# JiuTongBro/vqnerf_release

Hardware: AMD Instinct MI355X
Metric: rays/sec (render) 800x800, 64+64 samples/ray, NeuS SDF 8x256 + colour 4x256 (higher is better)
Workload: dtype f32; 1 GPU; BASELINE configs[1], nerf/hotdog-shaped NeuS render: one whole 800x800 pin-hole view per rank per step (camera at distance 4, fov 0.6911), n_samples=64, n_importance=64, up_sample_steps=4, sdf 8x256; parallelism=views x1 (no data-path collective)

## Files before the change

vqnerf_release_amd/csrc/neus_mlp.hip:

```cpp
#include "neus_launch.h"
#include <stdlib.h>

using namespace eng;

#ifdef VQN_STAMPS
__device__ unsigned long long g_stamps[8];
#define VQN_STAMP_DECL unsigned long long st_[6] = {0, 0, 0, 0, 0, 0}; unsigned long long st_prev = __builtin_amdgcn_s_memtime(); const unsigned long long st_begin = st_prev;
#define VQN_STAMP(i) { const unsigned long long st_now = __builtin_amdgcn_s_memtime(); st_[i] += st_now - st_prev; st_prev = st_now; }
#define VQN_STAMP_FLUSH if (threadIdx.x == 0) { st_[5] = __builtin_amdgcn_s_memtime() - st_begin; for (int i_ = 0; i_ < 6; ++i_) atomicAdd(&g_stamps[i_], st_[i_]); atomicAdd(&g_stamps[6], 1ull); }
extern "C" int vqn_debug_read_stamps(unsigned long long* out, int reset) {
  if (hipMemcpyFromSymbol(out, HIP_SYMBOL(g_stamps), sizeof(unsigned long long) * 8) != hipSuccess) return -3;
  if (reset) { unsigned long long z[8] = {0, 0, 0, 0, 0, 0, 0, 0}; if (hipMemcpyToSymbol(HIP_SYMBOL(g_stamps), z, sizeof(z)) != hipSuccess) return -3; }
  return 0;
}
#else
#define VQN_STAMP_DECL
#define VQN_STAMP(i)
#define VQN_STAMP_FLUSH
#endif

#ifdef VQN_STAMPS
__device__ unsigned long long g_stamps2[16];
#define FS_DECL unsigned long long fs_[16] = {0, 0, 0, 0, 0, 0, 0, 0, 0, 0, 0, 0, 0, 0, 0, 0}; unsigned long long fs_prev = __builtin_amdgcn_s_memtime(); const unsigned long long fs_begin = fs_prev;
#define FS(i) { const unsigned long long fs_now = __builtin_amdgcn_s_memtime(); fs_[i] += fs_now - fs_prev; fs_prev = fs_now; }
#define FS_FLUSH if (threadIdx.x == 0) { fs_[14] = __builtin_amdgcn_s_memtime() - fs_begin; for (int i_ = 0; i_ < 15; ++i_) atomicAdd(&g_stamps2[i_], fs_[i_]); atomicAdd(&g_stamps2[15], 1ull); }
extern "C" int vqn_debug_read_stamps2(unsigned long long* out, int reset) {
  if (hipMemcpyFromSymbol(out, HIP_SYMBOL(g_stamps2), sizeof(unsigned long long) * 16) != hipSuccess) return -3;
  if (reset) { unsigned long long z[16] = {0}; if (hipMemcpyToSymbol(HIP_SYMBOL(g_stamps2), z, sizeof(z)) != hipSuccess) return -3; }
  return 0;
}
#else
#define FS_DECL
#define FS(i)
#define FS_FLUSH
#endif

namespace {

constexpr int E0 = 0;
constexpr int E_ROWS = 8;

template <bool FINE>
__global__ __launch_bounds__(256, 2) void neus_points_kernel(
    const SdfDesc sd, const ColDesc cd, const f32x4* __restrict__ wsdf, const f32x4* __restrict__ wcol,
    const float* __restrict__ rays_o, const float* __restrict__ rays_d, const float* __restrict__ zv,
    const float* __restrict__ pts_direct, const float* __restrict__ dirs_direct, const long P, const int S,
    f32x4* __restrict__ scratch, float* __restrict__ out_sdf, float* __restrict__ out_grad,
    float* __restrict__ out_rgb) {
  extern __shared__ __attribute__((aligned(16))) f32x4 lds[];
  const int MT = sd.max_tiles;
  const int X0 = E_ROWS, Y0 = E_ROWS + 4 * MT;
  Smalls<1>* sm = reinterpret_cast<Smalls<1>*>(lds + (size_t)(E_ROWS + 8 * MT) * 64);
  const int tid = threadIdx.x, lane = tid & 63, h = lane >> 5, p = lane & 31;
  const int wave = __builtin_amdgcn_readfirstlane(tid >> 6);
  const int n_lin = sd.n_lin;
  const int emb_tiles = (sd.emb_feats + 31) >> 5;
  const long n_tiles = (P + 31) >> 5;
  f32x4* save = FINE ? scratch + (size_t)blockIdx.x * (size_t)(n_lin - 1) * 4 * MT * 64 : nullptr;
  const int feat_slot = (n_lin - 2) * 4 * MT;

  VQN_STAMP_DECL
  for (long tile = blockIdx.x; tile < n_tiles; tile += gridDim.x) {
    const long p0 = tile << 5;
    VQN_STAMP(4)
    if (tid < 32)
      load_point<FINE>(p0 + tid, P, S, rays_o, rays_d, zv, pts_direct, dirs_direct, sm->pts[0] + tid * 3, sm->dirs[0] + tid * 3);
    __syncthreads();
    const float xs = sm->pts[0][p * 3 + 0] * sd.scale, ys = sm->pts[0][p * 3 + 1] * sd.scale, zs = sm->pts[0][p * 3 + 2] * sd.scale;
    for (int r = wave; r < sd.emb_rows; r += 4) {
      f32x4 v;
#pragma unroll
      for (int j = 0; j < 4; ++j) v[j] = emb_feat(row_feat(r, h, j), sd.emb_feats, xs, ys, zs);
      lds[(E0 + r) * 64 + lane] = v;
    }
    __syncthreads();

    VQN_STAMP(0)
    int cur = X0, oth = Y0;
    f32x4 pre[4];
    {
      const f32x4* wp0 = wsdf + sd.layers[0].w_off + (size_t)wave * sd.emb_rows * 64 + lane;
#pragma unroll
      for (int i = 0; i < 4; ++i) pre[i] = wp0[i * 64];
    }
    for (int l = 0; l < n_lin - 1; ++l) {
      const LayerDesc L = sd.layers[l];
      const f32x4* next_wp = nullptr;
      if (l + 1 < n_lin - 1)
        next_wp = wsdf + sd.layers[l + 1].w_off + (size_t)wave * (4 * L.n_out_tiles + ((l + 1 == sd.skip) ? sd.emb_rows : 0)) * 64 + lane;
      const KSegs ks = (l == 0) ? KSegs{E0, sd.emb_rows, 0, 0}
                                : KSegs{cur, 4 * sd.layers[l - 1].n_out_tiles, E0, (l == sd.skip) ? sd.emb_rows : 0};
      const int dst = (l == 0) ? X0 : oth;
      const bool do_save = FINE && (l < n_lin - 2);
      const f32x4* bp = wsdf + L.b_off;
      f32x4* sv = save + (size_t)l * 4 * MT * 64;
      gemm_tiles_chain(lds, ks, wsdf + L.w_off, L.n_out_tiles, wave, lane, pre, next_wp,
                 [&](int ot, f32x16& acc) { VQN_STAMP(2) init_bias(bp, ot, lane, acc); },
                 [&](int ot, const f32x16& acc) {
                   VQN_STAMP(1)
#pragma unroll
                   for (int rq = 0; rq < 4; ++rq) {
                     f32x4 v = acc_quad(acc, rq);
#pragma unroll
                     for (int j = 0; j < 4; ++j) v[j] = act_fwd<ACT_SOFTPLUS100>(v[j]);
                     lds[(dst + ot * 4 + rq) * 64 + lane] = v;
                     if (do_save) st_stream(sv + (ot * 4 + rq) * 64 + lane, v);
                   }
                 });
      VQN_STAMP(2)
      __syncthreads();
      VQN_STAMP(3)
      if (l == 0) { cur = X0; oth = Y0; } else { const int t = cur; cur = oth; oth = t; }
    }
    const int hid_rows = 4 * sd.layers[n_lin - 2].n_out_tiles;

    rowdot<1>(lds, cur, hid_rows, wsdf + sd.last_w_off, sm->part[0], wave, lane);
    if (FINE && sd.layers[n_lin - 1].n_out_tiles > 0) {
      const LayerDesc L = sd.layers[n_lin - 1];
      const f32x4* bp = wsdf + L.b_off;
      f32x4* sv = save + (size_t)feat_slot * 64;
      gemm_tiles(lds, KSegs{cur, hid_rows, 0, 0}, wsdf + L.w_off, L.n_out_tiles, wave, lane,
                 [&](int ot, f32x16& acc) { init_bias(bp, ot, lane, acc); },
                 [&](int ot, const f32x16& acc) {
#pragma unroll
                   for (int rq = 0; rq < 4; ++rq) st_stream(sv + (ot * 4 + rq) * 64 + lane, acc_quad(acc, rq));
                 });
    }
    __syncthreads();
    if (tid < 32 && p0 + tid < P) out_sdf[p0 + tid] = sdf_raw(sm->part[0], tid, sd.last_b_off, sd.last_bias, wsdf) / sd.scale;
    if (!FINE) { __syncthreads(); continue; }

    for (int r0 = wave; r0 < hid_rows; r0 += 32) {
      f32x4 v[8], wv[8];
#pragma unroll
      for (int c = 0; c < 8; ++c) {
        const int r = min(r0 + 4 * c, hid_rows - 1);
        v[c] = lds[(cur + r) * 64 + lane];
        wv[c] = wsdf[sd.last_w_off + r * 2 + h];
      }
#pragma unroll
      for (int c = 0; c < 8; ++c)
        if (r0 + 4 * c < hid_rows) {
#pragma unroll
          for (int j = 0; j < 4; ++j) v[c][j] = wv[c][j] * act_bwd_from_out<ACT_SOFTPLUS100>(v[c][j]);
          lds[(cur + r0 + 4 * c) * 64 + lane] = v[c];
        }
    }
    __syncthreads();
    for (int l = n_lin - 2; l >= 1; --l) {
      const LayerDesc L = sd.layers[l];
      const KSegs ks{cur, 4 * L.n_out_tiles, 0, 0};
      const f32x4* sv = save + (size_t)(l - 1) * 4 * MT * 64;
      const int dst = oth;
      f32x4 hv[4];
      gemm_tiles(lds, ks, wsdf + L.wT_off, sd.layers[l - 1].n_out_tiles, wave, lane,
                 [&](int ot, f32x16& acc) {
#pragma unroll
                   for (int rq = 0; rq < 4; ++rq) hv[rq] = ld_stream(sv + (ot * 4 + rq) * 64 + lane);
                   init_zero(acc);
                 },
                 [&](int ot, const f32x16& acc) {
#pragma unroll
                   for (int rq = 0; rq < 4; ++rq) {
                     f32x4 v = acc_quad(acc, rq);
#pragma unroll
                     for (int j = 0; j < 4; ++j) v[j] *= act_bwd_from_out<ACT_SOFTPLUS100>(hv[rq][j]);
                     lds[(dst + ot * 4 + rq) * 64 + lane] = v;
                   }
                 });
      if (l == sd.skip)
        gemm_tiles(lds, ks, wsdf + L.wTE_off, emb_tiles, wave, lane,
                   [&](int, f32x16& acc) { init_zero(acc); },
                   [&](int ot, const f32x16& acc) {
#pragma unroll
                     for (int rq = 0; rq < 4; ++rq) lds[(E0 + ot * 4 + rq) * 64 + lane] = acc_quad(acc, rq);
                   });
      __syncthreads();
      const int t = cur; cur = oth; oth = t;
    }
    {
      const LayerDesc L = sd.layers[0];
      const bool accumulate = sd.skip >= 1;
      gemm_tiles(lds, KSegs{cur, 4 * L.n_out_tiles, 0, 0}, wsdf + L.wTE_off, emb_tiles, wave, lane,
                 [&](int ot, f32x16& acc) {
                   if (accumulate) init_rows(lds + (E0 + ot * 4) * 64, lane, acc); else init_zero(acc);
                 },
                 [&](int ot, const f32x16& acc) {
#pragma unroll
                   for (int rq = 0; rq < 4; ++rq) lds[(E0 + ot * 4 + rq) * 64 + lane] = acc_quad(acc, rq);
                 });
    }
    __syncthreads();
    if (tid < 96) {
      const int pp = tid & 31, c = tid >> 5;
      const float g = embed_chain([&](int f) { return lds_feat(lds, E0, f, pp); }, c, sd.multires, sm->pts[0] + pp * 3, sd.scale);
      sm->grad[0][pp * 3 + c] = g;
      if (p0 + pp < P) out_grad[(p0 + pp) * 3 + c] = g;
    }
    __syncthreads();
    if (cd.n_lin == 0) continue;

    {
      const float px = sm->pts[0][p * 3 + 0], py = sm->pts[0][p * 3 + 1], pz = sm->pts[0][p * 3 + 2];
      const float dx = sm->dirs[0][p * 3 + 0], dy = sm->dirs[0][p * 3 + 1], dz = sm->dirs[0][p * 3 + 2];
      for (int r = wave; r < cd.extra_rows; r += 4) {
        f32x4 v;
#pragma unroll
        for (int j = 0; j < 4; ++j) v[j] = col_extra_feat(row_feat(r, h, j), px, py, pz, dx, dy, dz, sm->grad[0] + p * 3, cd.n_view_feats, cd.extra_feats);
        lds[(E0 + r) * 64 + lane] = v;
      }
      const f32x4* sv = save + (size_t)feat_slot * 64;
      const int feat_rows = 4 * sd.layers[n_lin - 1].n_out_tiles;
      for (int r0 = wave; r0 < feat_rows; r0 += 32) {
        f32x4 v[8];
#pragma unroll
        for (int c = 0; c < 8; ++c) v[c] = ld_stream(sv + min(r0 + 4 * c, feat_rows - 1) * 64 + lane);
#pragma unroll
        for (int c = 0; c < 8; ++c)
          if (r0 + 4 * c < feat_rows) lds[(X0 + r0 + 4 * c) * 64 + lane] = v[c];
      }
      __syncthreads();
      cur = X0; oth = Y0;
      int in_rows = feat_rows;
      for (int l = 0; l < cd.n_lin - 1; ++l) {
        const LayerDesc L = cd.layers[l];
        const KSegs ks{cur, in_rows, E0, l == 0 ? cd.extra_rows : 0};
        const f32x4* bp = wcol + L.b_off;
        const int dst = oth;
        gemm_tiles(lds, ks, wcol + L.w_off, L.n_out_tiles, wave, lane,
                   [&](int ot, f32x16& acc) { init_bias(bp, ot, lane, acc); },
                   [&](int ot, const f32x16& acc) {
#pragma unroll
                     for (int rq = 0; rq < 4; ++rq) {
                       f32x4 v = acc_quad(acc, rq);
#pragma unroll
                       for (int j = 0; j < 4; ++j) v[j] = act_fwd<ACT_RELU>(v[j]);
                       lds[(dst + ot * 4 + rq) * 64 + lane] = v;
                     }
                   });
        __syncthreads();
        const int t = cur; cur = oth; oth = t;
        in_rows = 4 * L.n_out_tiles;
      }
      rowdot<3>(lds, cur, in_rows, wcol + cd.last_w_off, sm->part[0], wave, lane);
      __syncthreads();
      if (tid < 96) {
        const int pp = tid & 31, o = tid >> 5;
        const float v = rgb_out(sm->part[0], pp, o, cd.last_b_off, cd.last_bias[o], cd.squeeze_out, wcol);
        if (p0 + pp < P) out_rgb[(p0 + pp) * 3 + o] = v;
      }
    }
    __syncthreads();
  }
  VQN_STAMP(4)
  VQN_STAMP_FLUSH
}

__device__ __forceinline__ void wte_split_k(f32x4* __restrict__ lds, const int IS, const int k_row0, const int ng,
                                            const f32x4* __restrict__ w, const int emb_tiles, const int tmp_row0, const int tmp_rows,
                                            const int e_row0, const bool accumulate, const int wave, const int lane) {
  const int KS = min(8, tmp_rows >> 2) / emb_tiles, gk = (ng + KS - 1) / KS;
  const int t = wave % emb_tiles, kq = wave / emb_tiles;
  if (kq < KS) {
    f32x16 acc0, acc1;
    init_zero(acc0); init_zero(acc1);
    const int g0 = kq * gk, g1 = min(ng, g0 + gk);
    const f32x4* __restrict__ wp = w + (size_t)t * ng * 64 + lane;
    for (int g = g0; g < g1; g += 8) {
      f32x4 a[8], p[8], q[8];
#pragma unroll
      for (int i = 0; i < 8; ++i) {
        const int gg = min(g + i, ng - 1), r = (k_row0 + gg) * 64 + lane;
        a[i] = wp[gg * 64]; p[i] = lds[r]; q[i] = lds[r + IS];
      }
#pragma unroll
      for (int i = 0; i < 8; ++i)
        if (g + i < g1) {
#pragma unroll
          for (int j = 0; j < 4; ++j) {
            acc0 = __builtin_amdgcn_mfma_f32_32x32x2f32(a[i][j], p[i][j], acc0, 0, 0, 0);
            acc1 = __builtin_amdgcn_mfma_f32_32x32x2f32(a[i][j], q[i][j], acc1, 0, 0, 0);
          }
        }
    }
#pragma unroll
    for (int rq = 0; rq < 4; ++rq) {
      lds[(tmp_row0 + wave * 4 + rq) * 64 + lane] = acc_quad(acc0, rq);
      lds[IS + (tmp_row0 + wave * 4 + rq) * 64 + lane] = acc_quad(acc1, rq);
    }
  }
  __syncthreads();
  for (int r = wave; r < 8 * emb_tiles; r += 8) {
    const int im = r / (4 * emb_tiles), er = r - im * 4 * emb_tiles, tt = er >> 2, rq = er & 3;
    f32x4* li = lds + (size_t)im * IS;
    f32x4 sum = li[(tmp_row0 + tt * 4 + rq) * 64 + lane];
    for (int k = 1; k < KS; ++k) sum += li[(tmp_row0 + (k * emb_tiles + tt) * 4 + rq) * 64 + lane];
    if (accumulate) sum += li[(e_row0 + er) * 64 + lane];
    li[(e_row0 + er) * 64 + lane] = sum;
  }
  __syncthreads();
}

template <bool FINE, bool TRAIN = false, bool FOLD = false>
__global__ __launch_bounds__(512, 1) void neus_points2_kernel(
    const SdfDesc sd, const ColDesc cd, const f32x4* __restrict__ wsdf, const f32x4* __restrict__ wcol,
    const float* __restrict__ rays_o, const float* __restrict__ rays_d, const float* __restrict__ zv,
    const float* __restrict__ pts_direct, const float* __restrict__ dirs_direct, const long P, const int S,
    f32x4* __restrict__ scratch, float* __restrict__ out_sdf, float* __restrict__ out_grad,
    float* __restrict__ out_rgb, const TrainOut to) {
  extern __shared__ __attribute__((aligned(16))) f32x4 lds[];
  const int MT = sd.max_tiles;
  const int IMG = E_ROWS + 8 * MT, IS = IMG * 64;
  const int X0 = E_ROWS, Y0 = E_ROWS + 4 * MT;
  Smalls<2>* sm = reinterpret_cast<Smalls<2>*>(lds + (size_t)2 * IS);
  const int tid = threadIdx.x, lane = tid & 63, h = lane >> 5, p = lane & 31;
  const int wave = __builtin_amdgcn_readfirstlane(tid >> 6);
  const int img = wave >> 2, w4 = wave & 3;
  f32x4* ldsi = lds + (size_t)img * IS;
  const int n_lin = sd.n_lin;
  const int emb_tiles = (sd.emb_feats + 31) >> 5;
  const long n_tiles = (P + 31) >> 5, n_pairs = (n_tiles + 1) >> 1;
  const size_t per_img = (size_t)(n_lin - 1) * 4 * MT * 64;
#ifdef VQN_DIAG_STASH_ROT
  f32x4* save0 = nullptr;
#else
  f32x4* save0 = FINE ? scratch + (size_t)blockIdx.x * 2 * per_img : nullptr;
#endif
  const int feat_slot = (n_lin - 2) * 4 * MT;
  constexpr bool fold = FOLD;
  static_assert(!FOLD || (FINE && !TRAIN), "the fold is an inference path: the backward and the weight gradients read OUTF");
  f32x4 pre[4];
  f32x4 nopre[4];

  FS_DECL
  for (long pair = blockIdx.x; pair < n_pairs; pair += gridDim.x) {
#ifdef VQN_DIAG_STASH_ROT
    if (FINE) save0 = scratch + ((size_t)((pair / gridDim.x) % VQN_DIAG_STASH_ROT) * gridDim.x + blockIdx.x) * 2 * per_img;
#endif
    FS(12)
    if (tid < 64) {
      const int im = tid >> 5, t = tid & 31;
      load_point<FINE>(((2 * pair + im) << 5) + t, P, S, rays_o, rays_d, zv, pts_direct, dirs_direct, sm->pts[im] + t * 3, sm->dirs[im] + t * 3);
    }
    __syncthreads();
    const float xs = sm->pts[img][p * 3 + 0] * sd.scale, ys = sm->pts[img][p * 3 + 1] * sd.scale, zs = sm->pts[img][p * 3 + 2] * sd.scale;
    const long ptile_w = 2 * pair + img;
    for (int r = w4; r < (TRAIN ? 4 * to.e_tiles : sd.emb_rows); r += 4) {
      f32x4 v;
#pragma unroll
      for (int j = 0; j < 4; ++j) v[j] = r < sd.emb_rows ? emb_feat(row_feat(r, h, j), sd.emb_feats, xs, ys, zs) : 0.f;
      if (r < sd.emb_rows) ldsi[(E0 + r) * 64 + lane] = v;
      if (TRAIN && ptile_w < n_tiles) tfmt_store_quad(to.E, ptile_w, to.e_tiles, r >> 2, r & 3, lane, v);
    }
    __syncthreads();

    FS(0)
    int cur = X0, oth = Y0;
    if (wave < sd.layers[0].n_out_tiles) {
      const f32x4* wp0 = wsdf + sd.layers[0].w_off + (size_t)wave * sd.emb_rows * 64 + lane;
#pragma unroll
      for (int i = 0; i < 4; ++i) pre[i] = wp0[min(i, sd.emb_rows - 1) * 64];
    }
    for (int l = 0; l < n_lin - 1; ++l) {
      const LayerDesc L = sd.layers[l];
      const f32x4* next_wp = nullptr;
      if (l + 1 < n_lin - 1 && wave < sd.layers[l + 1].n_out_tiles)
        next_wp = wsdf + sd.layers[l + 1].w_off + (size_t)wave * (4 * L.n_out_tiles + ((l + 1 == sd.skip) ? sd.emb_rows : 0)) * 64 + lane;
      const KSegs ks = (l == 0) ? KSegs{E0, sd.emb_rows, 0, 0}
                                : KSegs{cur, 4 * sd.layers[l - 1].n_out_tiles, E0, (l == sd.skip) ? sd.emb_rows : 0};
      const int dst = (l == 0) ? X0 : oth;
      const bool do_save = FINE && (l < n_lin - 2);
      const f32x4* bp = wsdf + L.b_off;
      float* const t_u = TRAIN ? to.U[l + 1] : nullptr;
      auto bias_init = [&](int ot, int im, f32x16& acc) { if (im == 0) { FS(2) } init_bias(bp, ot, lane, acc); };
      auto epi_rq = [&](int ot, int im, int rq, const f32x16& acc) {
        if (im == 0 && rq == 0) { FS(1) }
        f32x4* li = lds + (size_t)im * IS;
        f32x4* sv = save0 + (size_t)im * per_img + (size_t)l * 4 * MT * 64;
        f32x4 v = {acc[4 * rq], acc[4 * rq + 1], acc[4 * rq + 2], acc[4 * rq + 3]};
#pragma unroll
        for (int j = 0; j < 4; ++j) v[j] = act_fwd<ACT_SOFTPLUS100>(v[j]);
        li[(dst + ot * 4 + rq) * 64 + lane] = v;
        if (do_save) st_stream(sv + (ot * 4 + rq) * 64 + lane, v);
        if (TRAIN && 2 * pair + im < n_tiles) tfmt_store_quad(t_u, 2 * pair + im, L.n_out_tiles, ot, rq, lane, v);
      };
      gemm_tiles2<8>(lds, IS, ks, wsdf + L.w_off, L.n_out_tiles, wave, lane, pre, true, next_wp, bias_init, epi_rq);
      FS(2)
      __syncthreads();
      FS(3)
      if (l == 0) { cur = X0; oth = Y0; } else { const int t = cur; cur = oth; oth = t; }
    }
    const int hid_rows = 4 * sd.layers[n_lin - 2].n_out_tiles;

    rowdot<1>(ldsi, cur, hid_rows, wsdf + sd.last_w_off, sm->part[img], w4, lane);
    if (FINE && sd.layers[n_lin - 1].n_out_tiles > 0) {
      const LayerDesc L = sd.layers[n_lin - 1];
      const f32x4* bp = fold ? wcol + cd.reserved2 : wsdf + L.b_off;
      gemm_tiles2<8>(lds, IS, KSegs{cur, hid_rows, 0, 0}, fold ? wcol + cd.reserved1 : wsdf + L.w_off,
                     fold ? cd.layers[0].n_out_tiles : L.n_out_tiles, wave, lane, nopre, false, nullptr,
                     [&](int ot, int, f32x16& acc) { init_bias(bp, ot, lane, acc); },
                     [&](int ot, int im, int rq, const f32x16& acc) {
                       f32x4* sv = save0 + (size_t)im * per_img + (size_t)feat_slot * 64;
                       const f32x4 v = {acc[4 * rq], acc[4 * rq + 1], acc[4 * rq + 2], acc[4 * rq + 3]};
                       st_stream(sv + (ot * 4 + rq) * 64 + lane, v);
                       if (TRAIN && 2 * pair + im < n_tiles) {
                         float* base = to.OUTF + (2 * pair + im) * (long)to.outf_tiles * 1024;
#pragma unroll
                         for (int j = 0; j < 4; ++j) {
                           const int f = 32 * ot + 2 * (4 * rq + j) + h + 1;
                           if (f < 32 * to.outf_tiles) __builtin_nontemporal_store(v[j], base + f * 32 + p);
                         }
                       }
                     });
    }
    __syncthreads();
    if (tid < 64) {
      const int im = tid >> 5, t = tid & 31;
      const long pt = ((2 * pair + im) << 5) + t;
      if (pt < P) out_sdf[pt] = sdf_raw(sm->part[im], t, sd.last_b_off, sd.last_bias, wsdf) / sd.scale;
      if (TRAIN && 2 * pair + im < n_tiles) {
        float* base = to.OUTF + (2 * pair + im) * (long)to.outf_tiles * 1024;
        base[t] = sdf_raw(sm->part[im], t, sd.last_b_off, sd.last_bias, wsdf);
        for (int f = 32 * sd.layers[n_lin - 1].n_out_tiles + 1; f < 32 * to.outf_tiles; ++f) base[f * 32 + t] = 0.f;
      }
    }
    if (!FINE) { __syncthreads(); FS(4) continue; }
    FS(4)

    float* const t_gh_top = TRAIN ? to.GH[n_lin - 2] : nullptr;
    for (int r0 = w4; r0 < hid_rows; r0 += 32) {
      f32x4 v[8], wv[8];
#pragma unroll
      for (int c = 0; c < 8; ++c) {
        const int r = min(r0 + 4 * c, hid_rows - 1);
        v[c] = ldsi[(cur + r) * 64 + lane];
        wv[c] = wsdf[sd.last_w_off + r * 2 + h];
      }
#pragma unroll
      for (int c = 0; c < 8; ++c)
        if (r0 + 4 * c < hid_rows) {
#pragma unroll
          for (int j = 0; j < 4; ++j) v[c][j] = wv[c][j] * act_bwd_from_out<ACT_SOFTPLUS100>(v[c][j]);
          ldsi[(cur + r0 + 4 * c) * 64 + lane] = v[c];
          if (TRAIN && ptile_w < n_tiles)
            tfmt_store_quad(t_gh_top, ptile_w, sd.layers[n_lin - 2].n_out_tiles, (r0 + 4 * c) >> 2, (r0 + 4 * c) & 3, lane, v[c]);
        }
    }
    __syncthreads();
    FS(5)
    for (int l = n_lin - 2; l >= 1; --l) {
      const LayerDesc L = sd.layers[l];
      const KSegs ks{cur, 4 * L.n_out_tiles, 0, 0};
      const int dst = oth;
      if (l == sd.skip)
        wte_split_k(lds, IS, cur, 4 * L.n_out_tiles, wsdf + L.wTE_off, emb_tiles, oth, 4 * MT, E0, false, wave, lane);
      f32x4 hv[2][4];
      float* const t_gh = TRAIN ? to.GH[l - 1] : nullptr;
      const int gh_tiles = sd.layers[l - 1].n_out_tiles;
      gemm_tiles2<8>(lds, IS, ks, wsdf + L.wT_off, sd.layers[l - 1].n_out_tiles, wave, lane, nopre, false, nullptr,
                     [&](int ot, int im, f32x16& acc) {
                       if (im == 0) { FS(7) }
                       const f32x4* sv = save0 + (size_t)im * per_img + (size_t)(l - 1) * 4 * MT * 64;
#pragma unroll
                       for (int rq = 0; rq < 4; ++rq) hv[im][rq] = ld_stream(sv + (ot * 4 + rq) * 64 + lane);
                       init_zero(acc);
                     },
                     [&](int ot, int im, int rq, const f32x16& acc) {
                       if (im == 0 && rq == 0) { FS(6) }
                       f32x4* li = lds + (size_t)im * IS;
                       f32x4 v = {acc[4 * rq], acc[4 * rq + 1], acc[4 * rq + 2], acc[4 * rq + 3]};
#pragma unroll
                       for (int j = 0; j < 4; ++j) v[j] *= act_bwd_from_out<ACT_SOFTPLUS100>(hv[im][rq][j]);
                       li[(dst + ot * 4 + rq) * 64 + lane] = v;
                       if (TRAIN && 2 * pair + im < n_tiles) tfmt_store_quad(t_gh, 2 * pair + im, gh_tiles, ot, rq, lane, v);
                     });
      FS(7)
      __syncthreads();
      FS(8)
      const int t = cur; cur = oth; oth = t;
    }
    wte_split_k(lds, IS, cur, 4 * sd.layers[0].n_out_tiles, wsdf + sd.layers[0].wTE_off, emb_tiles, oth, 4 * MT, E0, sd.skip >= 1, wave, lane);
    FS(6)
    if (tid < 192) {
      const int im = tid / 96, r = tid - 96 * im, pp = r & 31, c = r >> 5;
      const f32x4* li = lds + (size_t)im * IS;
      const float g = embed_chain([&](int f) { return lds_feat(li, E0, f, pp); }, c, sd.multires, sm->pts[im] + pp * 3, sd.scale);
      sm->grad[im][pp * 3 + c] = g;
      const long pt = ((2 * pair + im) << 5) + pp;
      if (pt < P) out_grad[pt * 3 + c] = g;
    }
    __syncthreads();
    FS(9)
    if (cd.n_lin == 0) continue;

    {
      const float px = sm->pts[img][p * 3 + 0], py = sm->pts[img][p * 3 + 1], pz = sm->pts[img][p * 3 + 2];
      const float dx = sm->dirs[img][p * 3 + 0], dy = sm->dirs[img][p * 3 + 1], dz = sm->dirs[img][p * 3 + 2];
      for (int r = w4; r < (TRAIN ? 4 * to.extr_tiles : cd.extra_rows); r += 4) {
        f32x4 v;
#pragma unroll
        for (int j = 0; j < 4; ++j)
          v[j] = r < cd.extra_rows ? col_extra_feat(row_feat(r, h, j), px, py, pz, dx, dy, dz, sm->grad[img] + p * 3, cd.n_view_feats, cd.extra_feats) : 0.f;
        if (r < cd.extra_rows) ldsi[(E0 + r) * 64 + lane] = v;
        if (TRAIN && ptile_w < n_tiles) tfmt_store_quad(to.EXTR, ptile_w, to.extr_tiles, r >> 2, r & 3, lane, v);
      }
      const f32x4* sv = save0 + (size_t)img * per_img + (size_t)feat_slot * 64;
      const int feat_rows = 4 * sd.layers[n_lin - 1].n_out_tiles;
      for (int r0 = w4; r0 < (fold ? 0 : feat_rows); r0 += 32) {
        f32x4 v[8];
#pragma unroll
        for (int c = 0; c < 8; ++c) v[c] = ld_stream(sv + min(r0 + 4 * c, feat_rows - 1) * 64 + lane);
#pragma unroll
        for (int c = 0; c < 8; ++c)
          if (r0 + 4 * c < feat_rows) ldsi[(X0 + r0 + 4 * c) * 64 + lane] = v[c];
      }
      __syncthreads();
      FS(10)
      cur = X0; oth = Y0;
      int in_rows = feat_rows;
      if (fold) {
        const LayerDesc L = cd.layers[0];
        const int dst = oth;
        gemm_tiles2<8>(lds, IS, KSegs{E0, cd.extra_rows, 0, 0}, wcol + cd.reserved3, L.n_out_tiles, wave, lane, nopre, false, nullptr,
                       [&](int ot, int im, f32x16& acc) {
                         const f32x4* pp = save0 + (size_t)im * per_img + (size_t)feat_slot * 64 + ot * 256 + lane;
#pragma unroll
                         for (int rq = 0; rq < 4; ++rq) {
                           const f32x4 v = ld_stream(pp + rq * 64);
                           acc[4 * rq + 0] = v[0]; acc[4 * rq + 1] = v[1]; acc[4 * rq + 2] = v[2]; acc[4 * rq + 3] = v[3];
                         }
                       },
                       [&](int ot, int im, int rq, const f32x16& acc) {
                         f32x4* li = lds + (size_t)im * IS;
                         f32x4 v = {acc[4 * rq], acc[4 * rq + 1], acc[4 * rq + 2], acc[4 * rq + 3]};
#pragma unroll
                         for (int j = 0; j < 4; ++j) v[j] = act_fwd<ACT_RELU>(v[j]);
                         li[(dst + ot * 4 + rq) * 64 + lane] = v;
                       });
        __syncthreads();
        const int t = cur; cur = oth; oth = t;
        in_rows = 4 * L.n_out_tiles;
      }
      for (int l = fold ? 1 : 0; l < cd.n_lin - 1; ++l) {
        const LayerDesc L = cd.layers[l];
        const KSegs ks{cur, in_rows, E0, l == 0 ? cd.extra_rows : 0};
        const f32x4* bp = wcol + L.b_off;
        const int dst = oth;
        float* const t_c = TRAIN ? to.C[l + 1] : nullptr;
        gemm_tiles2<8>(lds, IS, ks, wcol + L.w_off, L.n_out_tiles, wave, lane, nopre, false, nullptr,
                       [&](int ot, int, f32x16& acc) { init_bias(bp, ot, lane, acc); },
                       [&](int ot, int im, int rq, const f32x16& acc) {
                         f32x4* li = lds + (size_t)im * IS;
                         f32x4 v = {acc[4 * rq], acc[4 * rq + 1], acc[4 * rq + 2], acc[4 * rq + 3]};
#pragma unroll
                         for (int j = 0; j < 4; ++j) v[j] = act_fwd<ACT_RELU>(v[j]);
                         li[(dst + ot * 4 + rq) * 64 + lane] = v;
                         if (TRAIN && 2 * pair + im < n_tiles) tfmt_store_quad(t_c, 2 * pair + im, L.n_out_tiles, ot, rq, lane, v);
                       });
        __syncthreads();
        const int t = cur; cur = oth; oth = t;
        in_rows = 4 * L.n_out_tiles;
      }
      FS(11)
      rowdot<3>(ldsi, cur, in_rows, wcol + cd.last_w_off, sm->part[img], w4, lane);
      __syncthreads();
      if (tid < 192) {
        const int im = tid / 96, r = tid - 96 * im, pp = r & 31, o = r >> 5;
        const float v = rgb_out(sm->part[im], pp, o, cd.last_b_off, cd.last_bias[o], cd.squeeze_out, wcol);
        const long pt = ((2 * pair + im) << 5) + pp;
        if (pt < P) out_rgb[pt * 3 + o] = v;
      }
    }
    __syncthreads();
  }
  FS(12)
  FS_FLUSH
}

template <int NIMG>
struct SmallsSdf {
  float pts[NIMG][96], dirs[NIMG][96], part[NIMG][128];
};

template <int NIMG>
__global__ __launch_bounds__(512, 1) void neus_pointsN_kernel(
    const SdfDesc sd, const f32x4* __restrict__ wsdf, const float* __restrict__ rays_o, const float* __restrict__ rays_d,
    const float* __restrict__ zv, const float* __restrict__ pts_direct, const long P, const int S, float* __restrict__ out_sdf) {
  extern __shared__ __attribute__((aligned(16))) f32x4 lds[];
  const int MT = sd.max_tiles;
  const int X0 = sd.emb_rows, IS = (sd.emb_rows + 4 * MT) * 64;
  SmallsSdf<NIMG>* sm = reinterpret_cast<SmallsSdf<NIMG>*>(lds + (size_t)NIMG * IS);
  const int tid = threadIdx.x, lane = tid & 63, h = lane >> 5, p = lane & 31;
  const int wave = __builtin_amdgcn_readfirstlane(tid >> 6);
  const int n_lin = sd.n_lin;
  const long n_tiles = (P + 31) >> 5, n_groups = (n_tiles + NIMG - 1) / NIMG;
  f32x4 pre[4];
  f32x16 acc[NIMG];

  for (long grp = blockIdx.x; grp < n_groups; grp += gridDim.x) {
    if (tid < 32 * NIMG) {
      const int im = tid >> 5, t = tid & 31;
      load_point<false>(((NIMG * grp + im) << 5) + t, P, S, rays_o, rays_d, zv, pts_direct, nullptr, sm->pts[im] + t * 3, sm->dirs[im] + t * 3);
    }
    __syncthreads();
    for (int u = wave; u < NIMG * sd.emb_rows; u += 8) {
      const int im = u / sd.emb_rows, r = u - im * sd.emb_rows;
      const float xs = sm->pts[im][p * 3 + 0] * sd.scale, ys = sm->pts[im][p * 3 + 1] * sd.scale, zs = sm->pts[im][p * 3 + 2] * sd.scale;
      f32x4 v;
#pragma unroll
      for (int j = 0; j < 4; ++j) v[j] = emb_feat(row_feat(r, h, j), sd.emb_feats, xs, ys, zs);
      lds[(size_t)im * IS + (E0 + r) * 64 + lane] = v;
    }
    __syncthreads();

    if (wave < sd.layers[0].n_out_tiles) {
      const f32x4* wp0 = wsdf + sd.layers[0].w_off + (size_t)wave * sd.emb_rows * 64 + lane;
#pragma unroll
      for (int i = 0; i < 4; ++i) pre[i] = wp0[min(i, sd.emb_rows - 1) * 64];
    }
    for (int l = 0; l < n_lin - 1; ++l) {
      const LayerDesc L = sd.layers[l];
      const f32x4* next_wp = nullptr;
      if (l + 1 < n_lin - 1 && wave < sd.layers[l + 1].n_out_tiles)
        next_wp = wsdf + sd.layers[l + 1].w_off + (size_t)wave * (4 * L.n_out_tiles + ((l + 1 == sd.skip) ? sd.emb_rows : 0)) * 64 + lane;
      const KSegs ks = (l == 0) ? KSegs{E0, sd.emb_rows, 0, 0}
                                : KSegs{X0, 4 * sd.layers[l - 1].n_out_tiles, E0, (l == sd.skip) ? sd.emb_rows : 0};
      const f32x4* bp = wsdf + L.b_off;
      gemm_tilesN<NIMG, 8>(lds, IS, ks, wsdf + L.w_off, L.n_out_tiles, wave, lane, pre, next_wp, acc,
                           [&](int ot, int, f32x16& a) { init_bias(bp, ot, lane, a); },
                           [&](int, int, int rq, f32x16& a) {
#pragma unroll
                             for (int j = 0; j < 4; ++j) a[4 * rq + j] = act_fwd<ACT_SOFTPLUS100>(a[4 * rq + j]);
                           });
      if (l > 0) __syncthreads();
      if (wave < L.n_out_tiles) {
#pragma unroll
        for (int im = 0; im < NIMG; ++im) {
#pragma unroll
          for (int rq = 0; rq < 4; ++rq) lds[(size_t)im * IS + (X0 + wave * 4 + rq) * 64 + lane] = acc_quad(acc[im], rq);
        }
      }
      __syncthreads();
    }
    const int hid_rows = 4 * sd.layers[n_lin - 2].n_out_tiles;

    for (int u = wave; u < 4 * NIMG; u += 8)
      rowdot<1>(lds + (size_t)(u >> 2) * IS, X0, hid_rows, wsdf + sd.last_w_off, sm->part[u >> 2], u & 3, lane);
    __syncthreads();
    if (tid < 32 * NIMG) {
      const int im = tid >> 5, t = tid & 31;
      const long pt = ((NIMG * grp + im) << 5) + t;
      if (pt < P) out_sdf[pt] = sdf_raw(sm->part[im], t, sd.last_b_off, sd.last_bias, wsdf) / sd.scale;
    }
    __syncthreads();
  }
}

int check_sdf_desc(const SdfDesc& d) {
  if (d.n_lin < 2 || d.n_lin > VQN_MAX_SDF_LAYERS) return 1;
  if (d.max_tiles < 1 || d.max_tiles > 16) return 2;
  if (d.emb_feats < 3 || d.emb_feats > 64 || d.emb_rows < 1 || d.emb_rows > 8) return 3;
  if (d.skip >= d.n_lin - 1 || d.skip == 0) return 4;
  for (int l = 0; l < d.n_lin; ++l)
    if (d.layers[l].n_out_tiles < 0 || d.layers[l].n_out_tiles > d.max_tiles) return 5;
  if (!(d.scale > 0.f)) return 6;
  return 0;
}

template <int NIMG>
size_t lds_bytes(int MT) { return (size_t)NIMG * (E_ROWS + 8 * MT) * 1024 + sizeof(Smalls<NIMG>); }

bool use_two_images(int MT) {
  static const bool forced32 = getenv("VQN_NEUS_TILE32") != nullptr;
  return !forced32 && MT >= 5 && lds_bytes<2>(MT) <= 160 * 1024;
}

template <int NIMG>
size_t lds_bytes_sdf(const SdfDesc& sd) { return (size_t)NIMG * (sd.emb_rows + 4 * sd.max_tiles) * 1024 + sizeof(SmallsSdf<NIMG>); }

constexpr int SDF_IMAGES_DEFAULT = 4;
int sdf_images(const SdfDesc& sd) {
  static const int cap = [] {
    const char* e = getenv("VQN_NEUS_SDF_IMAGES");
    const int v = e != nullptr ? atoi(e) : SDF_IMAGES_DEFAULT;
    return v >= 2 && v <= 4 ? v : SDF_IMAGES_DEFAULT;
  }();
  if (!use_two_images(sd.max_tiles)) return 1;
  if (sd.max_tiles <= 8) {
    if (cap >= 4 && lds_bytes_sdf<4>(sd) <= 160 * 1024) return 4;
    if (cap >= 3 && lds_bytes_sdf<3>(sd) <= 160 * 1024) return 3;
  }
  return 2;
}

template <int NIMG>
int launch_sdf_images(const char* fn, const SdfDesc& sd, const f32x4* ws, const float* rays_o, const float* rays_d, const float* z,
                      const float* pts, const int64_t P, const int S, float* out_sdf, void* stream) {
  return vqn_launch(fn, neus_pointsN_kernel<NIMG>, pair_grid((P + 31) / 32, NIMG, 0, 0), 512, lds_bytes_sdf<NIMG>(sd), stream, sd, ws,
                    rays_o, rays_d, z, pts, (long)P, S, out_sdf);
}

bool extras_rows_ok(const ColDesc& cd) { return cd.extra_rows >= 1 && cd.extra_rows <= 8; }

}

extern "C" int vqn_neus_sdf_points(const int32_t* sdf_desc, const float* wbuf_sdf, const float* rays_o,
                                   const float* rays_d, const float* z, const float* pts, int64_t P, int S,
                                   float* out_sdf, void* stream) {
  SdfDesc sd;
  const int rc = neus_sdf_args(__func__, sdf_desc, wbuf_sdf, rays_o, rays_d, z, pts, P, S, out_sdf, check_sdf_desc,
                               "invalid SDF network descriptor", &sd);
  if (rc != VQN_OK || P == 0) return rc;
  ColDesc cd;
  memset(&cd, 0, sizeof(cd));
  const long n_tiles = (P + 31) / 32;
  const f32x4* ws = reinterpret_cast<const f32x4*>(wbuf_sdf);
  const int images = sdf_images(sd);
  if (images == 4) return launch_sdf_images<4>(__func__, sd, ws, rays_o, rays_d, z, pts, P, S, out_sdf, stream);
  if (images == 3) return launch_sdf_images<3>(__func__, sd, ws, rays_o, rays_d, z, pts, P, S, out_sdf, stream);
  if (images == 2)
    return vqn_launch(__func__, neus_points2_kernel<false>, pair_grid(n_tiles, 2, 0, 0), 512, lds_bytes<2>(sd.max_tiles), stream, sd, cd, ws,
                      nullptr, rays_o, rays_d, z, pts, nullptr, (long)P, S, nullptr, out_sdf, nullptr, nullptr, TrainOut{});
  const size_t lds = lds_bytes<1>(sd.max_tiles);
  VQN_CHECK_SHAPE(lds <= 160 * 1024, "network too wide for LDS");
  return vqn_launch(__func__, neus_points_kernel<false>, pair_grid(n_tiles, 1, 0, 0), 256, lds, stream, sd, cd, ws, nullptr, rays_o, rays_d,
                    z, pts, nullptr, (long)P, S, nullptr, out_sdf, nullptr, nullptr);
}

extern "C" int vqn_neus_train_fwd(const int32_t* sdf_desc, const float* wbuf_sdf, const int32_t* col_desc, const float* wbuf_col,
                                  const float* pts, const float* dirs, int64_t P, void* scratch, int64_t scratch_bytes,
                                  float* const* tensors, int n_tensors, int e_tiles, int outf_tiles, int extr_tiles, float* out_sdf,
                                  float* out_n, float* out_rgb, void* stream) {
  VQN_CHECK_ARG(sdf_desc && wbuf_sdf && col_desc && wbuf_col && pts && dirs && scratch && tensors && out_sdf && out_n && out_rgb, "null pointer");
  VQN_CHECK_ARG(P >= 1, "P >= 1");
  SdfDesc sd;
  ColDesc cd;
  memcpy(&sd, sdf_desc, sizeof(SdfDesc));
  memcpy(&cd, col_desc, sizeof(ColDesc));
  VQN_CHECK_SHAPE(check_sdf_desc(sd) == 0, "invalid SDF network descriptor");
  VQN_CHECK_SHAPE(cd.n_lin >= 2 && cd.n_lin <= VQN_MAX_COL_LAYERS && cd.d_out == 3 && sd.layers[sd.n_lin - 1].n_out_tiles >= 1, "colour net");
  VQN_CHECK_SHAPE(use_two_images(sd.max_tiles), "the training forward kernel is the two-image form only");
  const int nL = sd.n_lin - 1, nC = cd.n_lin - 1;
  VQN_CHECK_ARG(n_tensors == 3 + 2 * nL + nC, "tensors: [E, OUTF, EXTR, U_1..U_nL, GH_0..GH_{nL-1}, C_1..C_nC]");
  VQN_CHECK_SHAPE(e_tiles * 4 >= sd.emb_rows && e_tiles <= 2 && extr_tiles * 4 >= cd.extra_rows && extr_tiles <= 2 &&
                  outf_tiles >= sd.layers[sd.n_lin - 1].n_out_tiles, "tile counts");
  for (int i = 0; i < n_tensors; ++i) VQN_CHECK_ARG(tensors[i] != nullptr, "null tensor pointer");
  const long grid = pair_grid((P + 31) / 32, 2, neus_stash_bytes(sd), scratch_bytes);
  VQN_CHECK_ARG(grid >= 1, "scratch too small (see vqn_neus_fine_scratch_bytes)");
  return vqn_launch(__func__, neus_points2_kernel<true, true>, grid, 512, lds_bytes<2>(sd.max_tiles), stream, sd, cd,
                    reinterpret_cast<const f32x4*>(wbuf_sdf), reinterpret_cast<const f32x4*>(wbuf_col), nullptr, nullptr, nullptr, pts, dirs,
                    (long)P, 1, reinterpret_cast<f32x4*>(scratch), out_sdf, out_n, out_rgb,
                    neus_train_out(tensors, nL, nC, e_tiles, outf_tiles, extr_tiles));
}

extern "C" int64_t vqn_neus_fine_scratch_bytes(const int32_t* sdf_desc) {
  if (!sdf_desc) return -1;
  SdfDesc sd;
  memcpy(&sd, sdf_desc, sizeof(SdfDesc));
  const int emb_rows = sd.emb_rows;
  if (emb_rows >= 1 && emb_rows <= 12) sd.emb_rows = 1;
  if (check_sdf_desc(sd) != 0) return -2;
#ifdef VQN_DIAG_STASH_ROT
  return (int64_t)VQN_DIAG_STASH_ROT * vqn_num_cus() * 2 * neus_stash_bytes(sd);
#else
  return (int64_t)vqn_num_cus() * 2 * neus_stash_bytes(sd);
#endif
}

extern "C" int vqn_neus_fine_points(const int32_t* sdf_desc, const float* wbuf_sdf, const int32_t* col_desc,
                                    const float* wbuf_col, const float* rays_o, const float* rays_d, const float* z,
                                    const float* pts, const float* dirs, int64_t P, int S, void* scratch,
                                    int64_t scratch_bytes, float* out_sdf, float* out_grad, float* out_rgb,
                                    void* stream) {
  SdfDesc sd;
  ColDesc cd;
  const int rc = neus_fine_args(__func__, sdf_desc, wbuf_sdf, col_desc, wbuf_col, rays_o, rays_d, z, pts, dirs, P, S, scratch, out_sdf,
                                out_grad, out_rgb, check_sdf_desc, "invalid SDF network descriptor", extras_rows_ok, &sd, &cd);
  if (rc != VQN_OK || P == 0) return rc;
  if (cd.n_lin != 0)
    VQN_CHECK_ARG((cd.reserved1 > 0 && cd.reserved2 > cd.reserved1 && cd.reserved3 > cd.reserved2) ||
                  (cd.reserved1 == 0 && cd.reserved2 == 0 && cd.reserved3 == 0), "col_desc: fold offsets (reserved1..3) inconsistent");
  const long n_tiles = (P + 31) / 32;
  const int64_t per_img = neus_stash_bytes(sd);
  const f32x4* ws = reinterpret_cast<const f32x4*>(wbuf_sdf);
  const f32x4* wc = reinterpret_cast<const f32x4*>(wbuf_col);
  if (use_two_images(sd.max_tiles)) {
    const bool fold = cd.n_lin != 0 && cd.reserved1 > 0;
#ifdef VQN_DIAG_STASH_ROT
    const long grid = pair_grid(n_tiles, 2, 0, 0);
    VQN_CHECK_ARG((int64_t)VQN_DIAG_STASH_ROT * grid * 2 * per_img <= scratch_bytes, "diag build: scratch must hold ROT regions per workgroup");
#else
    const long grid = pair_grid(n_tiles, 2, per_img, scratch_bytes);
#endif
    VQN_CHECK_ARG(grid >= 1, "scratch too small (see vqn_neus_fine_scratch_bytes)");
    return vqn_launch(__func__, fold ? neus_points2_kernel<true, false, true> : neus_points2_kernel<true>, grid, 512, lds_bytes<2>(sd.max_tiles),
                      stream, sd, cd, ws, wc, rays_o, rays_d, z, pts, dirs, (long)P, S, reinterpret_cast<f32x4*>(scratch), out_sdf, out_grad,
                      out_rgb, TrainOut{});
  }
  const size_t lds = lds_bytes<1>(sd.max_tiles);
  VQN_CHECK_SHAPE(lds <= 160 * 1024, "network too wide for LDS");
  const long grid = pair_grid(n_tiles, 1, per_img, scratch_bytes);
  VQN_CHECK_ARG(grid >= 1, "scratch too small (see vqn_neus_fine_scratch_bytes)");
  return vqn_launch(__func__, neus_points_kernel<true>, grid, 256, lds, stream, sd, cd, ws, wc, rays_o, rays_d, z, pts, dirs, (long)P, S,
                    reinterpret_cast<f32x4*>(scratch), out_sdf, out_grad, out_rgb);
}
```

vqnerf_release_amd/csrc/neus_phases.h:

```cpp
#pragma once
#include "mlp_prims.h"
#include "tfmt.h"
#include "vqn_neus_desc.h"

namespace eng {

template <int NIMG>
struct Smalls {
  float pts[NIMG][96], dirs[NIMG][96], part[NIMG][512], grad[NIMG][96];
};

template <bool FINE>
__device__ __forceinline__ void load_point(long pt, const long P, const int S, const float* __restrict__ rays_o,
                                           const float* __restrict__ rays_d, const float* __restrict__ zv,
                                           const float* __restrict__ pts_direct, const float* __restrict__ dirs_direct,
                                           float* pts3, float* dirs3) {
  if (pt >= P) pt = P - 1;
  float x, y, z, dx = 0.f, dy = 0.f, dz = 0.f;
  if (pts_direct != nullptr) {
    x = pts_direct[pt * 3 + 0]; y = pts_direct[pt * 3 + 1]; z = pts_direct[pt * 3 + 2];
    if (FINE) { dx = dirs_direct[pt * 3 + 0]; dy = dirs_direct[pt * 3 + 1]; dz = dirs_direct[pt * 3 + 2]; }
  } else {
    const long ray = pt / S;
    const float t = zv[pt];
    dx = rays_d[ray * 3 + 0]; dy = rays_d[ray * 3 + 1]; dz = rays_d[ray * 3 + 2];
    x = rays_o[ray * 3 + 0] + __fmul_rn(dx, t);
    y = rays_o[ray * 3 + 1] + __fmul_rn(dy, t);
    z = rays_o[ray * 3 + 2] + __fmul_rn(dz, t);
  }
  pts3[0] = x; pts3[1] = y; pts3[2] = z;
  dirs3[0] = dx; dirs3[1] = dy; dirs3[2] = dz;
}

__device__ __forceinline__ float emb_feat(const int f, const int emb_feats, const float xs, const float ys, const float zs) {
  return f < emb_feats ? posenc_feat(f, xs, ys, zs) : 0.f;
}


__device__ __forceinline__ float sdf_raw(const float* pr, const int t, const int last_b_off, const float last_bias, const f32x4* __restrict__ wsdf) {
  return ((pr[t] + pr[32 + t]) + (pr[64 + t] + pr[96 + t])) + (last_b_off > 0 ? wsdf[last_b_off][0] : last_bias);
}

template <class Feat>
__device__ __forceinline__ float embed_chain(const Feat G, const int c, const int multires, const float* pts3, const float scale) {
  const float x0 = pts3[0] * scale, x1 = pts3[1] * scale, x2 = pts3[2] * scale;
  float g = G(c);
  int cc;
  for (int k = 0; k < multires; ++k) {
    const int fs = 3 + 6 * k + c, fc = fs + 3;
    g = fmaf(G(fs), posenc_jac(fs, x0, x1, x2, &cc), g);
    g = fmaf(G(fc), posenc_jac(fc, x0, x1, x2, &cc), g);
  }
  return g;
}

__device__ __forceinline__ float col_extra_feat(const int f, const float px, const float py, const float pz, const float dx,
                                                const float dy, const float dz, const float* grad3, const int n_view_feats,
                                                const int extra_feats) {
  float val = 0.f;
  if (f < 3) val = f == 0 ? px : (f == 1 ? py : pz);
  else if (f < 3 + n_view_feats) val = posenc_feat(f - 3, dx, dy, dz);
  else if (f < extra_feats) val = grad3[f - 3 - n_view_feats];
  return val;
}

__device__ __forceinline__ float rgb_out(const float* pr, const int pp, const int o, const int last_b_off, const float last_bias_o,
                                         const int squeeze_out, const f32x4* __restrict__ wcol) {
  float v = ((pr[(0 * 32 + pp) * 3 + o] + pr[(1 * 32 + pp) * 3 + o]) + (pr[(2 * 32 + pp) * 3 + o] + pr[(3 * 32 + pp) * 3 + o])) +
            (last_b_off > 0 ? wcol[last_b_off][o] : last_bias_o);
  if (squeeze_out) v = 1.f / (1.f + expf(-v));
  return v;
}

struct TrainOut {
  float* E; float* OUTF; float* EXTR;
  float* U[VQN_MAX_SDF_LAYERS]; float* GH[VQN_MAX_SDF_LAYERS]; float* C[VQN_MAX_COL_LAYERS];
  int e_tiles, outf_tiles, extr_tiles;
};

}
```

Measured before the change: 282,700 rays/s.

## Prefetch next tile's points and embedding during colour MLP in fine inference

In the fine inference path, the next pair's sample points are fetched into registers at the start of the colour network and written to shared memory after its first barrier. The positional embedding and layer-0 weight fragments are then computed between colour layers, overlapping that work with the current tile's tail. A second partial-sum buffer is added so the end-of-loop barrier can be dropped outside training. Timing stamps are also added to the multi-image SDF kernel. This costs extra LDS and register pressure and adds ordering hazards on the shared point and embedding buffers.

```diff
diff --git a/vqnerf_release_amd/csrc/neus_mlp.hip b/vqnerf_release_amd/csrc/neus_mlp.hip
--- a/vqnerf_release_amd/csrc/neus_mlp.hip
+++ b/vqnerf_release_amd/csrc/neus_mlp.hip
@@ -332,35 +332,64 @@
   f32x4 pre[4];
   f32x4 nopre[4];
 
+  constexpr bool PIPE = FINE && !TRAIN;
+  float* const part_b = reinterpret_cast<float*>(sm + 1);
+  bool primed = false;
+  int pb = 0;
+  auto fetch = [&](long pr) {
+    int t = tid;
+    asm volatile("" : "+v"(t));
+    return fetch_point<FINE>(((2 * pr + ((t >> 5) & 1)) << 5) + (t & 31), P, S, rays_o, rays_d, zv, pts_direct, dirs_direct);
+  };
+  auto put_points = [&](const PointRegs& q) {
+    int t = tid;
+    asm volatile("" : "+v"(t));
+    if (t < 64) store_point(q, sm->pts[t >> 5] + (t & 31) * 3, sm->dirs[t >> 5] + (t & 31) * 3);
+  };
+  auto embed = [&](long pr) {
+    const float xs = sm->pts[img][p * 3 + 0] * sd.scale, ys = sm->pts[img][p * 3 + 1] * sd.scale, zs = sm->pts[img][p * 3 + 2] * sd.scale;
+    const long ptile = 2 * pr + img;
+    for (int r = w4; r < (TRAIN ? 4 * to.e_tiles : sd.emb_rows); r += 4) {
+      f32x4 v;
+#pragma unroll
+      for (int j = 0; j < 4; ++j) v[j] = r < sd.emb_rows ? emb_feat(row_feat(r, h, j), sd.emb_feats, xs, ys, zs) : 0.f;
+      if (r < sd.emb_rows) ldsi[(E0 + r) * 64 + lane] = v;
+      if (TRAIN && ptile < n_tiles) tfmt_store_quad(to.E, ptile, to.e_tiles, r >> 2, r & 3, lane, v);
+    }
+  };
+  auto layer0_fragments = [&]() {
+    if (wave < sd.layers[0].n_out_tiles) {
+      int ln = lane;
+      if (PIPE) asm volatile("" : "+v"(ln));
+      const f32x4* wp0 = wsdf + sd.layers[0].w_off + (size_t)wave * sd.emb_rows * 64 + ln;
+#pragma unroll
+      for (int i = 0; i < 4; ++i) pre[i] = wp0[min(i, sd.emb_rows - 1) * 64];
+    }
+  };
+
   FS_DECL
-  for (long pair = blockIdx.x; pair < n_pairs; pair += gridDim.x) {
+  for (long pair = blockIdx.x; pair < n_pairs; pair += gridDim.x, pb ^= 1) {
 #ifdef VQN_DIAG_STASH_ROT
     if (FINE) save0 = scratch + ((size_t)((pair / gridDim.x) % VQN_DIAG_STASH_ROT) * gridDim.x + blockIdx.x) * 2 * per_img;
 #endif
     FS(12)
-    if (tid < 64) {
-      const int im = tid >> 5, t = tid & 31;
-      load_point<FINE>(((2 * pair + im) << 5) + t, P, S, rays_o, rays_d, zv, pts_direct, dirs_direct, sm->pts[im] + t * 3, sm->dirs[im] + t * 3);
-    }
-    __syncthreads();
-    const float xs = sm->pts[img][p * 3 + 0] * sd.scale, ys = sm->pts[img][p * 3 + 1] * sd.scale, zs = sm->pts[img][p * 3 + 2] * sd.scale;
+    float* const part0 = !TRAIN && pb ? part_b : sm->part[0];
+    float* const part = part0 + img * 512;
     const long ptile_w = 2 * pair + img;
-    for (int r = w4; r < (TRAIN ? 4 * to.e_tiles : sd.emb_rows); r += 4) {
-      f32x4 v;
-#pragma unroll
-      for (int j = 0; j < 4; ++j) v[j] = r < sd.emb_rows ? emb_feat(row_feat(r, h, j), sd.emb_feats, xs, ys, zs) : 0.f;
-      if (r < sd.emb_rows) ldsi[(E0 + r) * 64 + lane] = v;
-      if (TRAIN && ptile_w < n_tiles) tfmt_store_quad(to.E, ptile_w, to.e_tiles, r >> 2, r & 3, lane, v);
-    }
-    __syncthreads();
+    if (!primed) {
+      if (tid < 64) {
+        const int im = tid >> 5, t = tid & 31;
+        load_point<FINE>(((2 * pair + im) << 5) + t, P, S, rays_o, rays_d, zv, pts_direct, dirs_direct, sm->pts[im] + t * 3, sm->dirs[im] + t * 3);
+      }
+      __syncthreads();
+      embed(pair);
+      __syncthreads();
+      layer0_fragments();
+    }
+    primed = false;
 
     FS(0)
     int cur = X0, oth = Y0;
-    if (wave < sd.layers[0].n_out_tiles) {
-      const f32x4* wp0 = wsdf + sd.layers[0].w_off + (size_t)wave * sd.emb_rows * 64 + lane;
-#pragma unroll
-      for (int i = 0; i < 4; ++i) pre[i] = wp0[min(i, sd.emb_rows - 1) * 64];
-    }
     for (int l = 0; l < n_lin - 1; ++l) {
       const LayerDesc L = sd.layers[l];
       const f32x4* next_wp = nullptr;
@@ -392,7 +421,7 @@
     }
     const int hid_rows = 4 * sd.layers[n_lin - 2].n_out_tiles;
 
-    rowdot<1>(ldsi, cur, hid_rows, wsdf + sd.last_w_off, sm->part[img], w4, lane);
+    rowdot<1>(ldsi, cur, hid_rows, wsdf + sd.last_w_off, part, w4, lane);
     if (FINE && sd.layers[n_lin - 1].n_out_tiles > 0) {
       const LayerDesc L = sd.layers[n_lin - 1];
       const f32x4* bp = fold ? wcol + cd.reserved2 : wsdf + L.b_off;
@@ -417,10 +446,10 @@
     if (tid < 64) {
       const int im = tid >> 5, t = tid & 31;
       const long pt = ((2 * pair + im) << 5) + t;
-      if (pt < P) out_sdf[pt] = sdf_raw(sm->part[im], t, sd.last_b_off, sd.last_bias, wsdf) / sd.scale;
+      if (pt < P) out_sdf[pt] = sdf_raw(part0 + im * 512, t, sd.last_b_off, sd.last_bias, wsdf) / sd.scale;
       if (TRAIN && 2 * pair + im < n_tiles) {
         float* base = to.OUTF + (2 * pair + im) * (long)to.outf_tiles * 1024;
-        base[t] = sdf_raw(sm->part[im], t, sd.last_b_off, sd.last_bias, wsdf);
+        base[t] = sdf_raw(part0 + im * 512, t, sd.last_b_off, sd.last_bias, wsdf);
         for (int f = 32 * sd.layers[n_lin - 1].n_out_tiles + 1; f < 32 * to.outf_tiles; ++f) base[f * 32 + t] = 0.f;
       }
     }
@@ -494,6 +523,9 @@
     if (cd.n_lin == 0) continue;
 
     {
+      const bool has_next = PIPE && pair + gridDim.x < n_pairs;
+      PointRegs nq;
+      if (PIPE) nq = fetch(pair + gridDim.x);
       const float px = sm->pts[img][p * 3 + 0], py = sm->pts[img][p * 3 + 1], pz = sm->pts[img][p * 3 + 2];
       const float dx = sm->dirs[img][p * 3 + 0], dy = sm->dirs[img][p * 3 + 1], dz = sm->dirs[img][p * 3 + 2];
       for (int r = w4; r < (TRAIN ? 4 * to.extr_tiles : cd.extra_rows); r += 4) {
@@ -515,6 +547,7 @@
           if (r0 + 4 * c < feat_rows) ldsi[(X0 + r0 + 4 * c) * 64 + lane] = v[c];
       }
       __syncthreads();
+      if (has_next) put_points(nq);
       FS(10)
       cur = X0; oth = Y0;
       int in_rows = feat_rows;
@@ -538,6 +571,7 @@
                          li[(dst + ot * 4 + rq) * 64 + lane] = v;
                        });
         __syncthreads();
+        if (has_next) { FS(11) embed(pair + gridDim.x); primed = true; FS(13) }
         const int t = cur; cur = oth; oth = t;
         in_rows = 4 * L.n_out_tiles;
       }
@@ -558,20 +592,22 @@
                          if (TRAIN && 2 * pair + im < n_tiles) tfmt_store_quad(t_c, 2 * pair + im, L.n_out_tiles, ot, rq, lane, v);
                        });
         __syncthreads();
+        if (!fold && l == 0 && has_next) { FS(11) embed(pair + gridDim.x); primed = true; FS(13) }
         const int t = cur; cur = oth; oth = t;
         in_rows = 4 * L.n_out_tiles;
       }
+      if (primed) layer0_fragments();
       FS(11)
-      rowdot<3>(ldsi, cur, in_rows, wcol + cd.last_w_off, sm->part[img], w4, lane);
+      rowdot<3>(ldsi, cur, in_rows, wcol + cd.last_w_off, part, w4, lane);
       __syncthreads();
       if (tid < 192) {
         const int im = tid / 96, r = tid - 96 * im, pp = r & 31, o = r >> 5;
-        const float v = rgb_out(sm->part[im], pp, o, cd.last_b_off, cd.last_bias[o], cd.squeeze_out, wcol);
+        const float v = rgb_out(part0 + im * 512, pp, o, cd.last_b_off, cd.last_bias[o], cd.squeeze_out, wcol);
         const long pt = ((2 * pair + im) << 5) + pp;
         if (pt < P) out_rgb[pt * 3 + o] = v;
       }
     }
-    __syncthreads();
+    if (TRAIN) __syncthreads();
   }
   FS(12)
   FS_FLUSH
@@ -597,7 +633,9 @@
   f32x4 pre[4];
   f32x16 acc[NIMG];
 
+  FS_DECL
   for (long grp = blockIdx.x; grp < n_groups; grp += gridDim.x) {
+    FS(12)
     if (tid < 32 * NIMG) {
       const int im = tid >> 5, t = tid & 31;
       load_point<false>(((NIMG * grp + im) << 5) + t, P, S, rays_o, rays_d, zv, pts_direct, nullptr, sm->pts[im] + t * 3, sm->dirs[im] + t * 3);
@@ -613,6 +651,7 @@
     }
     __syncthreads();
 
+    FS(0)
     if (wave < sd.layers[0].n_out_tiles) {
       const f32x4* wp0 = wsdf + sd.layers[0].w_off + (size_t)wave * sd.emb_rows * 64 + lane;
 #pragma unroll
@@ -627,12 +666,15 @@
                                 : KSegs{X0, 4 * sd.layers[l - 1].n_out_tiles, E0, (l == sd.skip) ? sd.emb_rows : 0};
       const f32x4* bp = wsdf + L.b_off;
       gemm_tilesN<NIMG, 8>(lds, IS, ks, wsdf + L.w_off, L.n_out_tiles, wave, lane, pre, next_wp, acc,
-                           [&](int ot, int, f32x16& a) { init_bias(bp, ot, lane, a); },
-                           [&](int, int, int rq, f32x16& a) {
+                           [&](int ot, int im, f32x16& a) { if (im == 0) { FS(2) } init_bias(bp, ot, lane, a); },
+                           [&](int, int im, int rq, f32x16& a) {
+                             if (im == 0 && rq == 0) { FS(1) }
 #pragma unroll
                              for (int j = 0; j < 4; ++j) a[4 * rq + j] = act_fwd<ACT_SOFTPLUS100>(a[4 * rq + j]);
                            });
+      FS(2)
       if (l > 0) __syncthreads();
+      FS(3)
       if (wave < L.n_out_tiles) {
 #pragma unroll
         for (int im = 0; im < NIMG; ++im) {
@@ -640,7 +682,9 @@
           for (int rq = 0; rq < 4; ++rq) lds[(size_t)im * IS + (X0 + wave * 4 + rq) * 64 + lane] = acc_quad(acc[im], rq);
         }
       }
-      __syncthreads();
+      FS(2)
+      __syncthreads();
+      FS(3)
     }
     const int hid_rows = 4 * sd.layers[n_lin - 2].n_out_tiles;
 
@@ -653,7 +697,10 @@
       if (pt < P) out_sdf[pt] = sdf_raw(sm->part[im], t, sd.last_b_off, sd.last_bias, wsdf) / sd.scale;
     }
     __syncthreads();
+    FS(4)
   }
+  FS(12)
+  FS_FLUSH
 }
 
 int check_sdf_desc(const SdfDesc& d) {
@@ -668,7 +715,9 @@
 }
 
 template <int NIMG>
-size_t lds_bytes(int MT) { return (size_t)NIMG * (E_ROWS + 8 * MT) * 1024 + sizeof(Smalls<NIMG>); }
+size_t lds_bytes(int MT) {
+  return (size_t)NIMG * (E_ROWS + 8 * MT) * 1024 + sizeof(Smalls<NIMG>) + (NIMG == 2 ? sizeof(float) * 2 * 512 : 0);
+}
 
 bool use_two_images(int MT) {
   static const bool forced32 = getenv("VQN_NEUS_TILE32") != nullptr;
diff --git a/vqnerf_release_amd/csrc/neus_phases.h b/vqnerf_release_amd/csrc/neus_phases.h
--- a/vqnerf_release_amd/csrc/neus_phases.h
+++ b/vqnerf_release_amd/csrc/neus_phases.h
@@ -10,26 +10,48 @@
   float pts[NIMG][96], dirs[NIMG][96], part[NIMG][512], grad[NIMG][96];
 };
 
+struct PointRegs { float x, y, z, dx, dy, dz; };
+struct PointAddr { long pt, ray; };
+
+__device__ __forceinline__ PointAddr point_addr(long pt, const long P, const int S, const float* __restrict__ pts_direct) {
+  if (pt >= P) pt = P - 1;
+  return PointAddr{pt, pts_direct != nullptr ? 0 : pt / S};
+}
 template <bool FINE>
-__device__ __forceinline__ void load_point(long pt, const long P, const int S, const float* __restrict__ rays_o,
-                                           const float* __restrict__ rays_d, const float* __restrict__ zv,
-                                           const float* __restrict__ pts_direct, const float* __restrict__ dirs_direct,
-                                           float* pts3, float* dirs3) {
-  if (pt >= P) pt = P - 1;
+__device__ __forceinline__ PointRegs fetch_point_at(const PointAddr a, const float* __restrict__ rays_o, const float* __restrict__ rays_d,
+                                                    const float* __restrict__ zv, const float* __restrict__ pts_direct,
+                                                    const float* __restrict__ dirs_direct) {
+  const long pt = a.pt, ray = a.ray;
   float x, y, z, dx = 0.f, dy = 0.f, dz = 0.f;
   if (pts_direct != nullptr) {
     x = pts_direct[pt * 3 + 0]; y = pts_direct[pt * 3 + 1]; z = pts_direct[pt * 3 + 2];
     if (FINE) { dx = dirs_direct[pt * 3 + 0]; dy = dirs_direct[pt * 3 + 1]; dz = dirs_direct[pt * 3 + 2]; }
   } else {
-    const long ray = pt / S;
     const float t = zv[pt];
     dx = rays_d[ray * 3 + 0]; dy = rays_d[ray * 3 + 1]; dz = rays_d[ray * 3 + 2];
     x = rays_o[ray * 3 + 0] + __fmul_rn(dx, t);
     y = rays_o[ray * 3 + 1] + __fmul_rn(dy, t);
     z = rays_o[ray * 3 + 2] + __fmul_rn(dz, t);
   }
-  pts3[0] = x; pts3[1] = y; pts3[2] = z;
-  dirs3[0] = dx; dirs3[1] = dy; dirs3[2] = dz;
+  return PointRegs{x, y, z, dx, dy, dz};
+}
+template <bool FINE>
+__device__ __forceinline__ PointRegs fetch_point(const long pt, const long P, const int S, const float* __restrict__ rays_o,
+                                                 const float* __restrict__ rays_d, const float* __restrict__ zv,
+                                                 const float* __restrict__ pts_direct, const float* __restrict__ dirs_direct) {
+  return fetch_point_at<FINE>(point_addr(pt, P, S, pts_direct), rays_o, rays_d, zv, pts_direct, dirs_direct);
+}
+__device__ __forceinline__ void store_point(const PointRegs& q, float* pts3, float* dirs3) {
+  pts3[0] = q.x; pts3[1] = q.y; pts3[2] = q.z;
+  dirs3[0] = q.dx; dirs3[1] = q.dy; dirs3[2] = q.dz;
+}
+
+template <bool FINE>
+__device__ __forceinline__ void load_point(long pt, const long P, const int S, const float* __restrict__ rays_o,
+                                           const float* __restrict__ rays_d, const float* __restrict__ zv,
+                                           const float* __restrict__ pts_direct, const float* __restrict__ dirs_direct,
+                                           float* pts3, float* dirs3) {
+  store_point(fetch_point<FINE>(pt, P, S, rays_o, rays_d, zv, pts_direct, dirs_direct), pts3, dirs3);
 }
 
 __device__ __forceinline__ float emb_feat(const int f, const int emb_feats, const float xs, const float ys, const float zs) {
```

After: 283,900 rays/s, median of 6. About the same (+0.4%).
